# kirilllzaitsev/vision_mtl

Hardware: AMD Instinct MI355X
Metric: images/sec fwd+bwd, basic model 128x256 (higher is better)
Workload: dtype f32

## Files before the change

### include/vmtl.h

```cpp
#ifndef VMTL_H
#define VMTL_H

#ifdef __cplusplus
extern "C" {
#endif

#define VMTL_ACT_NONE 0
#define VMTL_ACT_RELU 1
#define VMTL_ACT_HSWISH 2
#define VMTL_ACT_HSIGMOID 3
#define VMTL_ACT_SIGMOID 4

#define VMTL_PREC_FP32 0
#define VMTL_PREC_BF16 1

const char* vmtl_version(void);
const char* vmtl_last_error_string(void);
int vmtl_reload_env(void);
int vmtl_timestamp(long long* out, void* stream);


int vmtl_conv2d_fwd(const float* x, const float* wp, const float* bias, float* y, float* stats,
                    int B, int H, int W, int Cs, int Ho, int Wo, int ldy, int Nw, int Cout,
                    int KH, int KW, int stride, int pad, int act, int shuffle, void* stream);
// ... 34 lines not shown
                           const float* ez_x, const float* ez_mean, const float* ez_invstd, const float* ez_gamma,
                           const float* ez_beta, int ez_act, int M, int Ks, int ldy, int Nw, int Cout, void* stream);

int vmtl_conv2d_bnbwd(const float* x, const float* wp, float* y, float* stats, const float* ez_x, const float* ez_mean,
                      const float* ez_invstd, const float* ez_gamma, const float* ez_beta, int ez_act, int B, int H,
                      int W, int Cs, int Ho, int Wo, int ldy, int Nw, int Cout, int KH, int KW, int stride, int pad,
                      void* stream);
int vmtl_conv2d_bnbwd_p(const float* x, const float* wp, float* y, float* stats, const float* ez_x, const float* ez_mean,
                        const float* ez_invstd, const float* ez_gamma, const float* ez_beta, int ez_act, int B, int H,
                        int W, int Cs, int Ho, int Wo, int ldy, int Nw, int Cout, int KH, int KW, int stride, int pad,
                        int precision, void* stream);

int vmtl_conv2d_up2_fwd(const float* xl, const float* skip, const float* wp_eff, float* y, float* stats,
                        int B, int H2, int W2, int C0s, int C1s, int ldy, int Cout, void* stream);
int vmtl_conv2d_up2_fwd_p(const float* xl, const float* skip, const float* wp_eff, float* y, float* stats,
                          int B, int H2, int W2, int C0s, int C1s, int ldy, int Cout, int precision, void* stream);
int vmtl_conv2d_up2_stats_block(int B, int H2, int W2, int ldy);
int vmtl_conv2d_up2_ksplit(int B, int H2, int W2, int ldy, int Ktot);
int vmtl_conv2d_up2_fwd_ws(const float* xl, const float* skip, const float* wp_eff, float* y, float* ws, int B, int H2,
                           int W2, int C0s, int C1s, int ldy, int Cout, void* stream);
int vmtl_conv2d_up2_fwd_ws_p(const float* xl, const float* skip, const float* wp_eff, float* y, float* ws, int B, int H2,
                             int W2, int C0s, int C1s, int ldy, int Cout, int precision, void* stream);
int vmtl_conv2d_up2_halo(const float* xl, const float* skip, const float* wp_eff, float* y, float* stats,
                         int B, int H2, int W2, int C0s, int C1s, int ldy, int Cout, void* stream);
int vmtl_conv2d_up2_halo_supported(int B, int H2, int W2, int C0s, int C1s, int ldy, int Cout);
int vmtl_conv2d_up2_halo_stat_rows(int B, int H2, int W2, int C0s, int C1s, int ldy, int Cout);
int vmtl_conv2d_up2_halo_stat_block(int C0s, int C1s, int ldy, int Cout);
int vmtl_pack_up2_fwd(const float* w, float* dst, int Cout, int C0, int C0s, int C1, int C1s, void* stream);
int vmtl_pack_up2_dgrad(const float* w, float* dst, int Cout, int Cos, int C0, int Cin, void* stream);
int vmtl_unpack_up2(const float* slabs, float* grad, int Cout, int Cos, int C0, int Cin, int nslabs, void* stream);

int vmtl_conv2d_wgrad_splits(int M, int Nw, int Ktot);
int vmtl_conv2d_wgrad(const float* x, const float* dy, float* slabs, int splits, int B, int H, int W, int Cs,
                      int Ho, int Wo, int ldy, int Nw, int KH, int KW, int stride, int pad, void* stream);
int vmtl_conv2d_wgrad_p(const float* x, const float* dy, float* slabs, int splits, int B, int H, int W, int Cs,
                        int Ho, int Wo, int ldy, int Nw, int KH, int KW, int stride, int pad, int precision,
                        void* stream);

int vmtl_conv3x3_wgrad_small_supported(int Cs, int ldy, int W);
int vmtl_conv3x3_wgrad_small_slabs(int B, int H, int W);
int vmtl_conv3x3_wgrad_small(const float* x, const float* dy, float* slabs, int nslabs, int B, int H, int W, int Cs,
                             int ldy, int Nw, void* stream);


int vmtl_conv3x3_small_supported(int Cs, int Nw);
int vmtl_conv3x3_small_tiles(int B, int H, int W);
int vmtl_conv3x3_small_stat_rows(int B, int H, int W);
int vmtl_conv3x3_small_stat_block(int B, int H, int W);
int vmtl_conv3x3_small(const float* x, const float* x2, const float* pa, const float* pb, const float* pc,
                       int act_in, float* a_out, const float* wp, const float* bias, float* y, float* yb, int Ca,
                       float* stats, int ep_mode, const float* ez_x, const float* ez_mean, const float* ez_invstd,
                       const float* ez_gamma, const float* ez_beta, int ez_act, int B, int H, int W, int Cs, int ldy,
                       int Nw, int Cout, void* stream);

int vmtl_dwconv_fwd(const float* x, const float* wp, float* y, int B, int H, int W, int Cs, int Ho, int Wo,
                    int K, int stride, int pad, void* stream);
int vmtl_dwconv_bn_stats_rows(int M, int Cs);
int vmtl_dwconv_bn_stats_block(int M, int Cs);
int vmtl_dwconv_bn_fwd(const float* x, const float* coef_a, const float* coef_c, int act, const float* wp, float* y,
                       float* a_out, float* partial, int B, int H, int W, int Cs, int Ho, int Wo, int K, int stride,
                       int pad, void* stream);
int vmtl_dwconv_bwd_data(const float* dy, const float* wp, float* dx, int B, int H, int W, int Cs, int Ho,
                         int Wo, int K, int stride, int pad, void* stream);
int vmtl_dwconv_bwd_data_add(const float* dy, const float* wp, const float* addend, float* dx, int B, int H, int W,
                             int Cs, int Ho, int Wo, int K, int stride, int pad, void* stream);
int vmtl_dwconv_bwd_weight_rows(int M, int Cs);
int vmtl_dwconv_bwd_weight(const float* x, const float* dy, float* partial, float* dw, int B, int H, int W,
                           int C, int Cs, int Ho, int Wo, int K, int stride, int pad, void* stream);

int vmtl_pack_weights(const float* src, float* dst, int R1, int R0, int T, int C, int Cs, long long sr1,
                      long long sr0, long long st, long long sc, int flip, void* stream);
int vmtl_pack_weights_scaled(const float* src, float* dst, int R1, int R0, int T, int C, int Cs, long long sr1,
                             long long sr0, long long st, long long sc, int flip, const float* scale, int sstride,
                             int smode, void* stream);
int vmtl_unpack_weights_stitch(const float* packed, float* grad, const float* w, const float* scale, int sstride,
                               float* ds, float* work, int R0, int T, int C, int Cs, int nslabs, long long slab_stride,
                               int reduce_all, void* stream);
int vmtl_pack_desc_bytes(void);
int vmtl_pack_weights_batch(const void* descs, int n, long long total, void* stream);
int vmtl_pack_weights_slice(const float* src, float* dst, int R0, int T, int C, int group, long long sr0,
                            long long st, long long sc, int flip, void* stream);
int vmtl_unpack_weights(const float* packed, float* grad, int R1, int R0, int T, int C, int Cs,
                        long long sr1, long long sr0, long long st, long long sc, int flip, int nslabs,
                        long long slab_stride, void* stream);

int vmtl_reduce_rows(int M);
int vmtl_bn_stats(const float* x, int M, int C, int Cs, float* partial, int nblk_from_conv,
                  int rows_per_blk_from_conv, float eps, float momentum, float* running_mean, float* running_var, long long* num_batches_tracked,
                  float* save_mean, float* save_invstd, void* stream);
int vmtl_bn_eval_stats(const float* running_mean, const float* running_var, int C, int Cs, float eps,
                       float* save_mean, float* save_invstd, void* stream);
int vmtl_bn_stats_coef(const float* x, int M, int C, int Cs, float* partial, int nblk_from_conv,
                       int rows_per_blk_from_conv, float eps, float momentum, float* running_mean, float* running_var,
                       long long* num_batches_tracked, float* save_mean, float* save_invstd, const float* gamma,
                       const float* beta, float* coef_a, float* coef_c, void* stream);
int vmtl_bn_eval_stats_coef(const float* running_mean, const float* running_var, int C, int Cs, float eps,
                            float* save_mean, float* save_invstd, const float* gamma, const float* beta,
                            float* coef_a, float* coef_c, void* stream);
int vmtl_bn_apply(const float* x, const float* mean, const float* invstd, const float* gamma,
                  const float* beta, const float* mul, const float* res, float* y, long long M, int C,
                  int Cs, int act, void* stream);
int vmtl_bn_fuse_max_rows(void);
int vmtl_bn_apply_fused(const float* x, const float* partial, int nblk, int rows_per_blk, float eps, float momentum,
                        float* running_mean, float* running_var, long long* num_batches_tracked, float* save_mean,
                        float* save_invstd, const float* gamma, const float* beta, const float* mul, const float* res,
                        float* y, long long M, int C, int Cs, int act, void* stream);
// ... 93 lines not shown
```

### vision_mtl_amd/ops.py

```python
from __future__ import annotations

import contextlib
import os
import weakref

import torch

from ._lib import lib
from .precision import conv_prec_code

ACT_NONE, ACT_RELU, ACT_HSWISH, ACT_HSIGMOID, ACT_SIGMOID = 0, 1, 2, 3, 4
ACT_CODES = {None: 0, "none": 0, "relu": 1, "hardswish": 2, "hardsigmoid": 3, "sigmoid": 4}


def ceil4(c: int) -> int:
    return (c + 3) // 4 * 4


def _stream() -> int:
    return torch.cuda.current_stream().cuda_stream


def _req(t: torch.Tensor, name: str = "tensor") -> torch.Tensor:
    if not t.is_cuda:
# ... 371 lines not shown


FUSE_DW = os.environ.get("VMTL_FUSE_DW", "1") != "0"
_PW = os.environ.get("VMTL_PW", "1") != "0"
_PW_MAX_ROWS = int(os.environ.get("VMTL_PW_MAX_ROWS", str(1 << 21)))


_UP2_HALO = os.environ.get("VMTL_UP2_HALO", "1") != "0"


def _up2_halo_route(B, H2, W2, C0s, C1s, ldy, Cout, prec) -> bool:
    return (_UP2_HALO and prec == 0 and bool(lib().raw("vmtl_conv2d_up2_halo_supported")(B, H2, W2, C0s, C1s, ldy, Cout))
            and lib().raw("vmtl_conv2d_up2_ksplit")(B, H2, W2, ldy, 4 * C0s + 9 * C1s) == 1)


def up2_stats_geometry(B, H2, W2, C0s, C1s, ldy, Cout, prec=None):
    prec = conv_prec_code() if prec is None else prec
    if _up2_halo_route(B, H2, W2, C0s, C1s, ldy, Cout, prec):
        return (lib().raw("vmtl_conv2d_up2_halo_stat_rows")(B, H2, W2, C0s, C1s, ldy, Cout),
                lib().raw("vmtl_conv2d_up2_halo_stat_block")(C0s, C1s, ldy, Cout))
    if lib().raw("vmtl_conv2d_up2_ksplit")(B, H2, W2, ldy, 4 * C0s + 9 * C1s) > 1:
        return 0, 0
    bm = lib().raw("vmtl_conv2d_up2_stats_block")(B, H2, W2, ldy)
    Mq = B * H2 * W2
    return (4 * (Mq // bm), bm) if Mq % bm == 0 else (0, bm)


def _is_pw(B, Ho, Wo, KH, KW, stride, pad, shuffle=0):
    return _PW and KH == 1 and KW == 1 and stride == 1 and pad == 0 and not shuffle and B * Ho * Wo <= _PW_MAX_ROWS


_SMALL_MIN_ROWS = int(os.environ.get("VMTL_SMALL_MIN_ROWS", str(1 << 16)))


def conv_ksplit(B, Ho, Wo, Cs, ldy, KH, KW, stride, pad, shuffle=0) -> int:
    if shuffle or _is_pw(B, Ho, Wo, KH, KW, stride, pad, shuffle):
        return 1
    return lib().raw("vmtl_conv2d_ksplit")(B, Ho, Wo, ldy, KH * KW * Cs)


_SMALL_STATS = os.environ.get("VMTL_SMALL_STATS", "1") != "0"


def _small_route(B, H, W, Cs, ldy, KH, KW, stride, pad, shuffle=0, with_stats=False) -> bool:
    if shuffle or KH != 3 or KW != 3 or stride != 1 or pad != 1 or ldy > 36 or B * H * W < _SMALL_MIN_ROWS:
        return False
    if B * H * W * 36 > 0x7FFFFFFF:
        return False
    if not conv3x3_small_supported(Cs, ldy):
        return False
    return not with_stats or (_SMALL_STATS and H % 4 == 0 and W % 32 == 0)


def conv_stats_geometry(B, Ho, Wo, Cs, ldy, KH, KW, stride, pad):
    if _small_route(B, Ho, Wo, Cs, ldy, KH, KW, stride, pad, with_stats=True):
        return lib().raw("vmtl_conv3x3_small_stat_rows")(B, Ho, Wo), lib().raw("vmtl_conv3x3_small_stat_block")(B, Ho, Wo)
    if _is_pw(B, Ho, Wo, KH, KW, stride, pad):
        M = B * Ho * Wo
        return lib().raw("vmtl_conv1x1_stats_rows")(M, ldy, Cs, 0), lib().raw("vmtl_conv1x1_stats_block")(M, ldy, Cs, 0)
    return lib().raw("vmtl_conv2d_stats_rows")(B, Ho, Wo, ldy), lib().raw("vmtl_conv2d_stats_block")(B, Ho, Wo, ldy)


def _conv_launch(x, wp, bias, y, stats, B, H, W, Cs, Ho, Wo, ldy, Nw, Cout, KH, KW, stride, pad, shuffle=0, cin=None,
                 algo_flop=None, prec=0):
    flop = 2.0 * B * Ho * Wo * Nw * KH * KW * (Cs if cin is None else cin)
    if _is_pw(B, Ho, Wo, KH, KW, stride, pad, shuffle):
        _k("vmtl_conv1x1_fwd", _flop=flop if algo_flop is None else algo_flop, _xflop=flop, x=x, wp=wp, bias=bias, y=y,
           stats=stats, M=B * Ho * Wo, Ks=Cs, ldy=ldy, Nw=Nw, Cout=Cout)
        return
    if _small_route(B, H, W, Cs, ldy, KH, KW, stride, pad, shuffle, with_stats=stats is not None):
        _small(x, wp, y, B, H, W, Cs, ldy, Nw, Cout, flop if algo_flop is None else algo_flop, bias=bias, stats=stats,
               ep_mode=1 if stats is not None else 0)
        return
    if stats is None and not shuffle:
        ks = lib().raw("vmtl_conv2d_ksplit")(B, Ho, Wo, ldy, KH * KW * Cs)
        if ks > 1:
            ws = _empty((ks, B * Ho * Wo, ldy), x)
            _kp("vmtl_conv2d_fwd_ws", prec, _flop=flop if algo_flop is None else algo_flop, _xflop=flop, x=x, wp=wp, bias=bias, y=y,
               ws=ws, B=B, H=H, W=W, Cs=Cs, Ho=Ho, Wo=Wo, ldy=ldy, Nw=Nw, Cout=Cout, KH=KH, KW=KW, stride=stride, pad=pad)
            return
    _kp("vmtl_conv2d_fwd", prec, _flop=flop if algo_flop is None else algo_flop, _xflop=flop, x=x, wp=wp, bias=bias, y=y, stats=stats, B=B, H=H, W=W, Cs=Cs, Ho=Ho, Wo=Wo, ldy=ldy,
       Nw=Nw, Cout=Cout, KH=KH, KW=KW, stride=stride, pad=pad, act=0, shuffle=shuffle)


def _stitch_view(stitch_w, task, C):
    T = stitch_w.shape[0]
    if stitch_w.dim() == 3:
        if stitch_w.shape[2] != C:
            raise ValueError(f"stitched conv: the stitch layer has {stitch_w.shape[2]} channels, the conv reads {C}")
        return (task * T + task) * C, 1
    return task * T + task, 0


class _Conv2d(torch.autograd.Function):

    @staticmethod
    def forward(ctx, x, weight, bias, stride, pad, want_stats, zero_bias_grad=False, stitch_w=None, stitch_task=0):
        x = _req(x, "x")
        weight = _req(weight, "weight")
        B, H, W, Cs = x.shape
        Cout, Cin, KH, KW = weight.shape
        if ceil4(Cin) != Cs:
            raise ValueError(f"conv2d: input has {Cs} storage channels, weight expects Cin={Cin}")
        KK = KH * KW
        Ho = (H + 2 * pad - KH) // stride + 1
        Wo = (W + 2 * pad - KW) // stride + 1
        ldy = ceil4(Cout)
        if stitch_w is None:
            wp = packs.get(weight, "fwd", (1, Cout, KK, Cin, Cs, 0, Cin * KK, 1, KK, 0))
        else:
            stitch_w = _req(stitch_w, "stitch weights")
            soff, sstride = _stitch_view(stitch_w, stitch_task, Cin)
            wp = packs.get(weight, f"fwd_st{stitch_task}", (1, Cout, KK, Cin, Cs, 0, Cin * KK, 1, KK, 0),
                           scale=(stitch_w, soff, sstride, 1))
        y = _empty((B, Ho, Wo, ldy), x)
        stats = None
        if want_stats and conv_ksplit(B, Ho, Wo, Cs, ldy, KH, KW, stride, pad) > 1:
            want_stats = False
        if want_stats:
            rows, _ = conv_stats_geometry(B, Ho, Wo, Cs, ldy, KH, KW, stride, pad)
            stats = _empty((rows, 2, ldy), x)
        prec = ctx.prec = conv_prec_code()
        _conv_launch(x, wp, bias, y, stats, B, H, W, Cs, Ho, Wo, ldy, Cout, Cout, KH, KW, stride, pad, cin=Cin, prec=prec)
        ctx.save_for_backward(x, weight, stitch_w)
        ctx.cfg = (stride, pad, bias is not None)
# ... 306 lines not shown

    @staticmethod
    def backward(ctx, dy, _dstats):
        xl, skip, weight = ctx.saved_tensors
        C0, C1, _ = ctx.cfg
        if dy is None:
            return None, None, None, None
        dy = _req(dy, "dy")
        B, H2, W2, C0s = xl.shape
        Cout, Cin = weight.shape[0], weight.shape[1]
        H, W, ldy = 2 * H2, 2 * W2, dy.shape[3]
        dxl = dskip = dw = None
        stamp(f"main up2 M={B * H * W} N={Cout} Cin={Cin}")
        fork = side.mark()
        if ctx.needs_input_grad[0]:
            wd = packs.get_custom(weight, "up2_dgrad", (C0, 16 * ldy), lambda w, dst: _k(
                "vmtl_pack_up2_dgrad", w=w, dst=dst, Cout=Cout, Cos=ldy, C0=C0, Cin=Cin))
            dxl = _empty((B, H2, W2, C0s), xl)
            _conv_launch(dy, wd, None, dxl, None, B, H, W, ldy, H2, W2, C0s, C0, C0, 4, 4, 2, 1, cin=Cout,
                         algo_flop=2.0 * B * H * W * C0 * 9 * Cout, prec=ctx.prec)
        if skip is not None and ctx.needs_input_grad[1]:
            C1s = skip.shape[3]
            wds = packs.get(weight, "up2_dskip", (1, C1, 9, Cout, ldy, 0, 9, 1, Cin * 9, 1), offset=C0 * 9)
            dskip = _empty((B, H, W, C1s), xl)
            _conv_launch(dy, wds, None, dskip, None, B, H, W, ldy, H, W, C1s, C1, C1, 3, 3, 1, 1, cin=Cout, prec=ctx.prec)
        if ctx.needs_input_grad[2]:
            dw = _empty(weight.shape, xl) if ctx.slot is None else ctx.slot
            with side.branch(ctx.slot is not None, B * H * W, fork, dy, xl, skip):
                slabs, ns = _wgrad(dy, xl, B, H, W, ldy, H2, W2, C0s, C0, 4, 4, 2, 1, 2.0 * B * H * W * Cout * 9 * C0,
                                   xflop=2.0 * B * H2 * W2 * C0 * 16 * Cout, prec=ctx.prec)
                _k("vmtl_unpack_up2", slabs=slabs, grad=dw, Cout=Cout, Cos=ldy, C0=C0, Cin=Cin, nslabs=ns)
                if skip is not None:
                    C1s = skip.shape[3]
                    slabs, ns = _wgrad(skip, dy, B, H, W, C1s, H, W, ldy, Cout, 3, 3, 1, 1,
                                       2.0 * B * H * W * Cout * 9 * C1, prec=ctx.prec)
                    unpack(slabs, None, 1, Cout, 9, C1, C1s, 0, Cin * 9, 1, 9, out=dw.view(-1)[C0 * 9:], nslabs=ns)
                stamp(f"side up2 M={B * H * W} N={Cout} Cin={Cin}")
            if ctx.slot is not None:
                dw = None
        return dxl, dskip, dw, None, None


class _BNActConv(torch.autograd.Function):

    @staticmethod
    def forward(ctx, x, stats, rpb, gamma, beta, rm, rv, nbt, weight, skip, cfg):
        C, training, momentum, eps, act, up2, want_stats = cfg
        x, weight = _req(x, "x"), _req(weight, "weight")
        B, H, W, Cs = x.shape
        M = B * H * W
        Cout, Cin = weight.shape[0], weight.shape[1]
        if ceil4(C) != Cs or tuple(weight.shape[2:]) != (3, 3):
            raise ValueError("bn_act_conv: 3x3 weight over x's channels expected")
        mean, invstd = _empty((Cs,), x), _empty((Cs,), x)
        a = _empty(x.shape, x)
        if training:
            if stats is not None:
                partial, nblk = stats, stats.shape[0]
            else:
                partial, nblk, rpb = _empty((_reduce_rows(M), 2, Cs), x), 0, 0
            if 0 < nblk <= _BN_FUSE_ROWS:
                _k("vmtl_bn_apply_fused", x=x, partial=partial, nblk=nblk, rows_per_blk=rpb, eps=eps, momentum=momentum,
                   running_mean=rm, running_var=rv, num_batches_tracked=nbt, save_mean=mean, save_invstd=invstd,
                   gamma=gamma, beta=beta, mul=None, res=None, y=a, M=M, C=C, Cs=Cs, act=act)
            else:
                _k("vmtl_bn_stats", x=x, M=M, C=C, Cs=Cs, partial=partial, nblk_from_conv=nblk, rows_per_blk_from_conv=rpb,
                   eps=eps, momentum=momentum, running_mean=rm, running_var=rv, num_batches_tracked=nbt, save_mean=mean,
                   save_invstd=invstd)
                _k("vmtl_bn_apply", x=x, mean=mean, invstd=invstd, gamma=gamma, beta=beta, mul=None, res=None, y=a, M=M,
                   C=C, Cs=Cs, act=act)
        else:
            _k("vmtl_bn_eval_stats", running_mean=rm, running_var=rv, C=C, Cs=Cs, eps=eps, save_mean=mean, save_invstd=invstd)
            _k("vmtl_bn_apply", x=x, mean=mean, invstd=invstd, gamma=gamma, beta=beta, mul=None, res=None, y=a, M=M, C=C,
               Cs=Cs, act=act)
        prec = ctx.prec = conv_prec_code()
        ldy = ceil4(Cout)
        ostats, orpb = None, 0
        if up2:
            if skip is not None:
                skip = _req(skip, "skip")
                C1s = skip.shape[3]
                if tuple(skip.shape[:3]) != (B, 2 * H, 2 * W):
                    raise ValueError("bn_act_conv(up2): skip must be at twice the resolution of x")
            else:
                C1s = 0
            C1 = Cin - C
            if ceil4(C1) != C1s or (C1 > 0) != (skip is not None):
                raise ValueError("bn_act_conv(up2): weight channels do not match x + skip")
            Ktot = 4 * Cs + 9 * C1s
            wp = packs.get_custom(weight, "up2_fwd", (4, Cout, Ktot), lambda w, dst: _k(
                "vmtl_pack_up2_fwd", w=w, dst=dst, Cout=Cout, C0=C, C0s=Cs, C1=C1, C1s=C1s))
            y = _empty((B, 2 * H, 2 * W, ldy), x)
            Mo = 4 * M
            ks = lib().raw("vmtl_conv2d_up2_ksplit")(B, H, W, ldy, Ktot)
            if _up2_halo_route(B, H, W, Cs, C1s, ldy, Cout, prec):
                if want_stats:
                    rows, bm = up2_stats_geometry(B, H, W, Cs, C1s, ldy, Cout, prec)
                    if rows:
                        ostats, orpb = _empty((rows, 2, ldy), x), bm
                _k("vmtl_conv2d_up2_halo", _flop=2.0 * Mo * Cout * 9 * Cin, _xflop=2.0 * Mo * Cout * (4 * C + 9 * C1), xl=a,
                   skip=skip, wp_eff=wp, y=y, stats=ostats, B=B, H2=H, W2=W, C0s=Cs, C1s=C1s, ldy=ldy, Cout=Cout)
            elif ks > 1:
                _kp("vmtl_conv2d_up2_fwd_ws", prec, _flop=2.0 * Mo * Cout * 9 * Cin, _xflop=2.0 * Mo * Cout * (4 * C + 9 * C1),
                   xl=a, skip=skip, wp_eff=wp, y=y, ws=_empty((ks, B, 2 * H, 2 * W, ldy), x), B=B, H2=H, W2=W, C0s=Cs,
                   C1s=C1s, ldy=ldy, Cout=Cout)
            else:
                if want_stats:
                    bm = lib().raw("vmtl_conv2d_up2_stats_block")(B, H, W, ldy)
                    if M % bm == 0:
                        ostats, orpb = _empty((4 * (M // bm), 2, ldy), x), bm
                _kp("vmtl_conv2d_up2_fwd", prec, _flop=2.0 * Mo * Cout * 9 * Cin, _xflop=2.0 * Mo * Cout * (4 * C + 9 * C1), xl=a,
                   skip=skip, wp_eff=wp, y=y, stats=ostats, B=B, H2=H, W2=W, C0s=Cs, C1s=C1s, ldy=ldy, Cout=Cout)
        else:
            if Cin != C or skip is not None:
                raise ValueError("bn_act_conv: weight expects x's channels (skip only with up2)")
            wp = packs.get(weight, "fwd", (1, Cout, 9, Cin, Cs, 0, Cin * 9, 1, 9, 0))
            y = _empty((B, H, W, ldy), x)
            if want_stats and conv_ksplit(B, H, W, Cs, ldy, 3, 3, 1, 1) == 1:
                rows, orpb = conv_stats_geometry(B, H, W, Cs, ldy, 3, 3, 1, 1)
                ostats = _empty((rows, 2, ldy), x)
            _conv_launch(a, wp, None, y, ostats, B, H, W, Cs, H, W, ldy, Cout, Cout, 3, 3, 1, 1, cin=Cin, prec=prec)
        ctx.save_for_backward(x, a, skip, weight, mean, invstd, gamma, beta)
        ctx.cfg = (C, training, act, up2)
        ctx.slots = (_slot(gamma), _slot(beta), _slot(weight))
        ctx.orpb = orpb
        ctx.set_materialize_grads(False)
        if ostats is not None:
            ctx.mark_non_differentiable(ostats)
        return y, ostats

    @staticmethod
    def backward(ctx, dy, _dstats):
        x, a, skip, weight, mean, invstd, gamma, beta = ctx.saved_tensors
        C, training, act, up2 = ctx.cfg
        sg, sb, sw = ctx.slots
        if dy is None:
            return (None,) * 11
        dy = _req(dy, "dy")
        B, H, W, Cs = x.shape
        M = B * H * W
        Cout, Cin = weight.shape[0], weight.shape[1]
        ldy = dy.shape[3]
        stamp(f"main bnconv M={dy.shape[0] * dy.shape[1] * dy.shape[2]} N={Cout} Cin={Cin}")
        fork = side.mark()
        if up2:
            Hd, Wd = 2 * H, 2 * W
            wd = packs.get_custom(weight, "up2_dgrad", (C, 16 * ldy), lambda w, dst: _k(
                "vmtl_pack_up2_dgrad", w=w, dst=dst, Cout=Cout, Cos=ldy, C0=C, Cin=Cin))
            geo = dict(B=B, H=Hd, W=Wd, Cs=ldy, Ho=H, Wo=W, ldy=Cs, Nw=C, Cout=C, KH=4, KW=4, stride=2, pad=1)
            flop, xflop = 2.0 * B * Hd * Wd * C * 9 * Cout, 2.0 * M * C * 16 * Cout
        else:
            Hd, Wd = H, W
            wd = packs.get(weight, "dgrad", (1, Cin, 9, Cout, ldy, 0, 9, 1, Cin * 9, 1))
            geo = dict(B=B, H=H, W=W, Cs=ldy, Ho=H, Wo=W, ldy=Cs, Nw=Cin, Cout=Cin, KH=3, KW=3, stride=1, pad=1)
            flop = xflop = 2.0 * M * Cin * 9 * Cout
        dgamma = _empty((C,), x) if sg is None else sg
        dbeta = _empty((C,), x) if sb is None else sb
        dx = _empty(x.shape, x) if ctx.needs_input_grad[0] else None
        fuse = lib().raw("vmtl_conv2d_ksplit")(B, H, W, Cs, geo["KH"] * geo["KW"] * ldy) <= 1 \
            and os.environ.get("VMTL_BNBWD_FUSE", "1") != "0"
        if fuse:
            dz = _empty(x.shape, x)
            if not up2 and _small_route(B, H, W, ldy, Cs, 3, 3, 1, 1, with_stats=True):
                rows = lib().raw("vmtl_conv3x3_small_stat_rows")(B, H, W)
                part = _empty((rows, 2, Cs), x)
                _small(dy, wd, dz, B, H, W, ldy, Cs, Cin, Cin, flop, stats=part, ep_mode=2,
                       ez=(x, mean, invstd, gamma, beta, act))
            else:
                rows = lib().raw("vmtl_conv2d_stats_rows")(B, H, W, Cs)
                part = _empty((rows, 2, Cs), x)
                _kp("vmtl_conv2d_bnbwd", ctx.prec, _flop=flop, _xflop=xflop, x=dy, wp=wd, y=dz, stats=part, ez_x=x, ez_mean=mean,
                   ez_invstd=invstd, ez_gamma=gamma, ez_beta=beta, ez_act=act, **geo)
            _k("vmtl_bn_bwd_finalize", partial=part, nblk=rows, M=M, C=C, Cs=Cs, sum_dz=dbeta, sum_dzx=dgamma, mean=None,
               invstd=None, gamma=None, training=1 if training else 0, coef_a=None, coef_b=None, coef_c=None)
            if dx is not None:
                _k("vmtl_bn_bwd_apply", x=x, dz=dz, mean=mean, invstd=invstd, gamma=gamma, sum_dz=dbeta, sum_dzx=dgamma,
                   dx=dx, M=M, C=C, Cs=Cs, training=1 if training else 0)
        else:
            da = _empty(x.shape, x)
            _conv_launch(dy, wd, None, da, None, geo["B"], geo["H"], geo["W"], geo["Cs"], geo["Ho"], geo["Wo"], geo["ldy"],
                         geo["Nw"], geo["Cout"], geo["KH"], geo["KW"], geo["stride"], geo["pad"], cin=Cout, algo_flop=flop,
                         prec=ctx.prec)
            part = _empty((_reduce_rows(M), 2, Cs), x)
            _k("vmtl_bn_bwd", x=x, dy=da, mean=mean, invstd=invstd, gamma=gamma, beta=beta, mul=None, dmul=None,
               partial=part, sum_dz=dbeta, sum_dzx=dgamma, dx=dx if dx is not None else _empty(x.shape, x), M=M, C=C, Cs=Cs,
               act=act, training=1 if training else 0)
        dskip = None
        if up2 and skip is not None and ctx.needs_input_grad[9]:
            C1, C1s = Cin - C, skip.shape[3]
            wds = packs.get(weight, "up2_dskip", (1, C1, 9, Cout, ldy, 0, 9, 1, Cin * 9, 1), offset=C * 9)
            dskip = _empty(skip.shape, x)
            _conv_launch(dy, wds, None, dskip, None, B, Hd, Wd, ldy, Hd, Wd, C1s, C1, C1, 3, 3, 1, 1, cin=Cout, prec=ctx.prec)
        dw = _empty(weight.shape, x) if sw is None else sw
        with side.branch(sw is not None, B * Hd * Wd, fork, dy, a, skip):
            if up2:
                slabs, ns = _wgrad(dy, a, B, Hd, Wd, ldy, H, W, Cs, C, 4, 4, 2, 1, 2.0 * B * Hd * Wd * Cout * 9 * C,
                                   xflop=2.0 * M * C * 16 * Cout, prec=ctx.prec)
                _k("vmtl_unpack_up2", slabs=slabs, grad=dw, Cout=Cout, Cos=ldy, C0=C, Cin=Cin, nslabs=ns)
                if skip is not None:
                    C1, C1s = Cin - C, skip.shape[3]
                    slabs, ns = _wgrad(skip, dy, B, Hd, Wd, C1s, Hd, Wd, ldy, Cout, 3, 3, 1, 1,
                                       2.0 * B * Hd * Wd * Cout * 9 * C1, prec=ctx.prec)
                    unpack(slabs, None, 1, Cout, 9, C1, C1s, 0, Cin * 9, 1, 9, out=dw.view(-1)[C * 9:], nslabs=ns)
            else:
                slabs, ns = _wgrad(a, dy, B, H, W, Cs, H, W, ldy, Cout, 3, 3, 1, 1, 2.0 * M * Cout * 9 * Cin, prec=ctx.prec)
                unpack(slabs, weight.shape, 1, Cout, 9, Cin, Cs, 0, Cin * 9, 1, 9, out=dw, nslabs=ns)
            stamp(f"side bnconv N={Cout} Cin={Cin}")
        nif = lambda g, slot: None if slot is not None else g
        return dx, None, None, nif(dgamma, sg), nif(dbeta, sb), None, None, None, nif(dw, sw), dskip, None


def bn_act_conv(x, stats, rpb, bn, C, act, weight, skip=None, up2=False, want_stats=True):
    if bn.momentum is None:
        raise NotImplementedError("BatchNorm2d(momentum=None) (cumulative moving average) is not implemented")
    cfg = (C, bn.training, float(bn.momentum), bn.eps, act, bool(up2), bool(want_stats))
    y, ostats = _BNActConv.apply(x, stats, rpb, bn.weight, bn.bias, bn.running_mean, bn.running_var,
                                 bn.num_batches_tracked, weight, skip, cfg)
    orpb = 0
    if ostats is not None:
        B, H, W, _ = x.shape
# ... 1173 lines not shown
```

Measured before the change: 2592.

## Add halo-tiled MFMA 3x3 conv kernel with fused BN prologue and stats epilogue

Adds a new 3x3 stride-1 conv kernel for 64/68 input channels. It stages a haloed 4x32 pixel tile of the input in LDS, runs fp32 MFMA with a software-pipelined weight prefetch, and writes BN statistics or the BN-backward dz epilogue from the output tile. The BN->act->conv forward path now applies the BN affine and ReLU inside the conv prologue and writes the activation as a side output, which removes the separate bn_apply pass. The kernel is routed for mid-size fp32 convs in forward, the generic conv launcher and BN backward. In exchange it adds a large new code path with several template variants and extra LDS use.

```diff
diff --git a/include/vmtl.h b/include/vmtl.h
--- a/include/vmtl.h
+++ b/include/vmtl.h
@@ -110,6 +110,14 @@
                        float* stats, int ep_mode, const float* ez_x, const float* ez_mean, const float* ez_invstd,
                        const float* ez_gamma, const float* ez_beta, int ez_act, int B, int H, int W, int Cs, int ldy,
                        int Nw, int Cout, void* stream);
+
+int vmtl_conv3x3_halo_supported(int B, int H, int W, int Cs, int ldy, int Nw);
+int vmtl_conv3x3_halo_stat_rows(int B, int H, int W);
+int vmtl_conv3x3_halo_stat_block(int B, int H, int W);
+int vmtl_conv3x3_halo(const float* x, const float* pa, const float* pc, int act_in, float* a_out, const float* wp,
+                      const float* bias, float* y, float* stats, int ep_mode, const float* ez_x, const float* ez_mean,
+                      const float* ez_invstd, const float* ez_gamma, const float* ez_beta, int ez_act, int B, int H,
+                      int W, int Cs, int ldy, int Nw, int Cout, void* stream);
 
 int vmtl_dwconv_fwd(const float* x, const float* wp, float* y, int B, int H, int W, int Cs, int Ho, int Wo,
                     int K, int stride, int pad, void* stream);
diff --git a/vision_mtl_amd/csrc/conv3x3_halo.hip b/vision_mtl_amd/csrc/conv3x3_halo.hip
--- /dev/null
+++ b/vision_mtl_amd/csrc/conv3x3_halo.hip
@@ -0,0 +1,392 @@
+#include "common.h"
+
+#define CH_TM 4
+#define CH_TW 32
+#define CH_HX (CH_TW + 2)
+#define CH_NHALO ((CH_TM + 2) * CH_HX)
+#define CH_NP (CH_NHALO | 1)
+#define CH_NPX (CH_TM * CH_TW)
+
+struct HaloP {
+  const float* x;
+  const float* pa;
+  const float* pc;
+  float* a_out;
+  const float* wp;
+  const float* bias;
+  float* y;
+  float* stats;
+  const float* ez_x;
+  const float* ez_mean;
+  const float* ez_invstd;
+  const float* ez_gamma;
+  const float* ez_beta;
+  int act_in, ep_mode, ez_act;
+  int B, H, W, ldy, Nw, Cout;
+  int tiles_x, tiles_y;
+  unsigned x_bytes, wp_bytes;
+};
+
+template <int CS, int TN, bool TAIL>
+struct HaloCfg {
+  static constexpr int SP = CS / 4, FG = SP / 4, RS = SP % 4;
+  static constexpr int KQ = 9 * SP;
+  static constexpr int NGF = 9 * FG, NR = 9 * RS, NGR = (NR + 3) / 4;
+  static constexpr int NG = NGF + NGR;
+  static constexpr int NROWS = 16 * TN;
+  static constexpr int OS = NROWS + 4;
+  static constexpr int SQ = TAIL ? OS / 4 : TN * 4;
+  static constexpr int NRT = 2 * CH_TM;
+  static constexpr int WM = 4 / TN;
+  static constexpr int RT = NRT / WM;
+  static constexpr int NST = CH_NHALO * SP;
+  static constexpr int IT = (NST + 255) / 256;
+  static constexpr int ZQ = SP * CH_NP;
+  static constexpr int HALO4 = ZQ + 1;
+  static constexpr int OT4 = CH_NPX * OS / 4;
+  static constexpr int RED4 = 2 * 256;
+  static constexpr int MAIN4 = HALO4 > OT4 + RED4 ? HALO4 : OT4 + RED4;
+  static constexpr int PQ = (OS + 3) / 4;
+  static constexpr int PAR4 = 2 * SP + 5 * PQ;
+  static constexpr int LDS_BYTES = (MAIN4 + PAR4) * 16;
+  static_assert(TN == 1 || TN == 2 || TN == 4, "column tiles");
+  static_assert(!TAIL || TN == 4, "tail columns only next to 4 MFMA column tiles (one per wave)");
+  static_assert(CS % 4 == 0 && FG >= 1, "channel quads");
+};
+
+__device__ __forceinline__ f32x4 ch_bload(__amdgpu_buffer_rsrc_t r, unsigned off) {
+  return __builtin_bit_cast(f32x4, __builtin_amdgcn_raw_buffer_load_b128(r, off, 0, 0));
+}
+
+template <int CS, int TN, bool TAIL>
+__global__ __launch_bounds__(256) __attribute__((amdgpu_waves_per_eu(2))) void conv3x3_halo_kernel(HaloP p) {
+  using C = HaloCfg<CS, TN, TAIL>;
+  constexpr int SP = C::SP, FG = C::FG, RS = C::RS, KQ = C::KQ, NGF = C::NGF, NR = C::NR, NGR = C::NGR, NG = C::NG;
+  constexpr int NROWS = C::NROWS, OS = C::OS, RT = C::RT, IT = C::IT, ZQ = C::ZQ, PQ = C::PQ;
+  constexpr int NB = TAIL ? 2 : 1;
+  constexpr unsigned OOB = 0xFFFFFFFFu;
+
+  extern __shared__ __attribute__((aligned(16))) f32x4 smem4[];
+  f32x4* halo = smem4;
+  float* otile = reinterpret_cast<float*>(smem4);
+  f32x4* red = smem4 + C::OT4;
+  f32x4* par = smem4 + C::MAIN4;
+  f32x4* epar = par + 2 * SP;
+
+  const int tid = threadIdx.x;
+  const int lane = tid & 63, wv = __builtin_amdgcn_readfirstlane(tid >> 6);
+  const int l15 = lane & 15, lq = lane >> 4;
+  const int jw = wv % TN, rw = wv / TN;
+
+  int t = blockIdx.x;
+  const int tx = t % p.tiles_x;
+  t /= p.tiles_x;
+  const int ty = t % p.tiles_y, b = t / p.tiles_y;
+  const int h0 = ty * CH_TM, w0 = tx * CH_TW;
+
+  const __amdgpu_buffer_rsrc_t rs_x = __builtin_amdgcn_make_buffer_rsrc((void*)p.x, 0, p.x_bytes, 0x00020000);
+  const __amdgpu_buffer_rsrc_t rs_w = __builtin_amdgcn_make_buffer_rsrc((void*)p.wp, 0, p.wp_bytes, 0x00020000);
+
+  const bool has_pro = p.pa != nullptr;
+  if (tid < 2 * SP) {
+    const float* src = tid < SP ? p.pa : p.pc;
+    const int s = tid < SP ? tid : tid - SP;
+    par[tid] = has_pro ? *reinterpret_cast<const f32x4*>(src + 4 * s) : (f32x4){0.f, 0.f, 0.f, 0.f};
+  }
+  if (tid < 5 * PQ) {
+    const int which = tid / PQ, q = tid - which * PQ;
+    const float* src = which == 0 ? p.bias : (which == 1 ? p.ez_mean : (which == 2 ? p.ez_invstd : (which == 3 ? p.ez_gamma : p.ez_beta)));
+    f32x4 v = {0.f, 0.f, 0.f, 0.f};
+    if (src != nullptr && (which == 0 || p.ep_mode == 2)) {
+#pragma unroll
+      for (int e = 0; e < 4; ++e)
+        if (4 * q + e < p.Cout) v[e] = src[4 * q + e];
+    }
+    epar[tid] = v;
+  }
+
+  unsigned wrow[NB];
+  {
+    const int n = 16 * jw + l15;
+    wrow[0] = n < p.Nw ? (unsigned)(n * KQ) * 16u : 0x80000000u;
+    if (TAIL) {
+      const int nt = NROWS + wv;
+      wrow[NB - 1] = nt < p.Nw ? (unsigned)(nt * KQ) * 16u : 0x80000000u;
+    }
+  }
+  int arem[NGR > 0 ? NGR : 1];
+  unsigned krem[NGR > 0 ? NGR : 1];
+#pragma unroll
+  for (int h = 0; h < NGR; ++h) {
+    const int r = 4 * h + lq;
+    if (r < NR) {
+      const int tap = r / (RS > 0 ? RS : 1), s = FG * 4 + r % (RS > 0 ? RS : 1);
+      arem[h] = s * CH_NP + (tap / 3) * CH_HX + tap % 3 + l15;
+      krem[h] = (unsigned)(tap * SP + s) * 16u;
+    } else {
+      arem[h] = -1;
+      krem[h] = 0x40000000u;
+    }
+  }
+  const int a0 = lq * CH_NP + l15;
+  auto rtoff = [](int i) { return (i >> 1) * CH_HX + 16 * (i & 1); };
+
+  {
+    f32x4 r0[IT];
+#pragma unroll
+    for (int it = 0; it < IT; ++it) {
+      const int f = tid + 256 * it;
+      const int pp = f / SP, s = f - pp * SP;
+      const int hy = pp / CH_HX, hx = pp - hy * CH_HX;
+      const int gh = h0 - 1 + hy, gw = w0 - 1 + hx;
+      const bool ok = f < C::NST && (unsigned)gh < (unsigned)p.H && (unsigned)gw < (unsigned)p.W;
+      r0[it] = ch_bload(rs_x, ok ? (unsigned)((b * p.H + gh) * p.W + gw) * (unsigned)(CS * 4) + 16u * s : OOB);
+    }
+    if (has_pro) __syncthreads();
+#pragma unroll
+    for (int it = 0; it < IT; ++it) {
+      const int f = tid + 256 * it;
+      if (f >= C::NST) continue;
+      const int pp = f / SP, s = f - pp * SP;
+      f32x4 v = r0[it];
+      if (has_pro) {
+        const int hy = pp / CH_HX, hx = pp - hy * CH_HX;
+        const int gh = h0 - 1 + hy, gw = w0 - 1 + hx;
+        const bool ok = (unsigned)gh < (unsigned)p.H && (unsigned)gw < (unsigned)p.W;
+        v = v * par[s] + par[SP + s];
+        if (p.act_in == VMTL_ACT_RELU) {
+#pragma unroll
+          for (int e = 0; e < 4; ++e) v[e] = fmaxf(v[e], 0.f);
+        }
+        if (!ok) v = (f32x4){0.f, 0.f, 0.f, 0.f};
+        if (p.a_out != nullptr && ok && hy >= 1 && hy <= CH_TM && hx >= 1 && hx <= CH_TW)
+          *reinterpret_cast<f32x4*>(p.a_out + (size_t)((b * p.H + gh) * p.W + gw) * CS + 4 * s) = v;
+      }
+      halo[s * CH_NP + pp] = v;
+    }
+    if (tid == 0) halo[ZQ] = (f32x4){0.f, 0.f, 0.f, 0.f};
+  }
+
+  constexpr int SQ = C::SQ, G = 256 / SQ;
+  constexpr int EIT = (CH_NPX + G - 1) / G;
+  const int eq = tid % SQ, gi = tid / SQ;
+  const bool elane = gi < G;
+  f32x4 rz[EIT];
+  if (p.ep_mode == 2) {
+#pragma unroll
+    for (int it = 0; it < EIT; ++it) {
+      const int px = gi + it * G;
+      const int gy = h0 + px / CH_TW, gx = w0 + px % CH_TW;
+      rz[it] = (f32x4){0.f, 0.f, 0.f, 0.f};
+      if (elane && px < CH_NPX && gy < p.H && gx < p.W)
+        rz[it] = *reinterpret_cast<const f32x4*>(p.ez_x + (size_t)((b * p.H + gy) * p.W + gx) * p.ldy + 4 * eq);
+    }
+  }
+  __syncthreads();
+
+  f32x4 acc[RT];
+  f32x2 tacc[TAIL ? C::NRT : 1];
+#pragma unroll
+  for (int i = 0; i < RT; ++i) acc[i] = (f32x4){0.f, 0.f, 0.f, 0.f};
+#pragma unroll
+  for (int i = 0; i < (TAIL ? C::NRT : 1); ++i) tacc[i] = (f32x2){0.f, 0.f};
+  const int rbase = rw * RT;
+  auto group = [&](int g, unsigned& koff, int& ai) {
+    if (g < NGF) {
+      const int tap = g / FG, cb = (g % FG) * 4;
+      koff = (unsigned)(tap * SP + cb + lq) * 16u;
+      ai = a0 + cb * CH_NP + (tap / 3) * CH_HX + tap % 3;
+    } else {
+      koff = krem[g - NGF];
+      ai = arem[g - NGF];
+    }
+  };
+  auto load_b = [&](int g, f32x4 (&bq)[NB]) {
+    unsigned koff;
+    int ai;
+    group(g, koff, ai);
+#pragma unroll
+    for (int j = 0; j < NB; ++j) bq[j] = ch_bload(rs_w, wrow[j] + koff);
+  };
+  auto load_a = [&](int g, f32x4 (&aq)[RT]) {
+    unsigned koff;
+    int ai;
+    group(g, koff, ai);
+#pragma unroll
+    for (int i = 0; i < RT; ++i) aq[i] = halo[ai < 0 ? ZQ : ai + rtoff(rbase + i)];
+  };
+  auto mma = [&](const f32x4 (&aq)[RT], const f32x4 (&bq)[NB]) {
+#pragma unroll
+    for (int e = 0; e < 4; ++e)
+#pragma unroll
+      for (int i = 0; i < RT; ++i) acc[i] = __builtin_amdgcn_mfma_f32_16x16x4f32(aq[i][e], bq[0][e], acc[i], 0, 0, 0);
+    if (TAIL) {
+      const f32x4 w = bq[NB - 1];
+      const f32x2 lo = __builtin_shufflevector(w, w, 0, 1), hi = __builtin_shufflevector(w, w, 2, 3);
+#pragma unroll
+      for (int i = 0; i < (TAIL ? C::NRT : 1); ++i) {
+        tacc[i] += __builtin_shufflevector(aq[i], aq[i], 0, 1) * lo;
+        tacc[i] += __builtin_shufflevector(aq[i], aq[i], 2, 3) * hi;
+        asm volatile("" : "+v"(tacc[i]));
+      }
+    }
+  };
+  f32x4 bq[3][NB], aq[2][RT];
+  load_b(0, bq[0]);
+  if (NG > 1) load_b(1, bq[1]);
+  load_a(0, aq[0]);
+#pragma unroll
+  for (int g = 0; g < NG; ++g) {
+    if (g + 2 < NG) load_b(g + 2, bq[(g + 2) % 3]);
+    if (g + 1 < NG) load_a(g + 1, aq[(g + 1) & 1]);
+    mma(aq[g & 1], bq[g % 3]);
+    if (g + 2 < NG) __builtin_amdgcn_sched_group_barrier(0x020, NB, 0);
+    if (g + 1 < NG) __builtin_amdgcn_sched_group_barrier(0x100, RT, 0);
+    __builtin_amdgcn_sched_group_barrier(0x008, 4 * RT, 0);
+    if (TAIL) __builtin_amdgcn_sched_group_barrier(0x002, 4 * C::NRT + 8, 0);
+    __builtin_amdgcn_sched_barrier(0);
+  }
+
+  float tv[TAIL ? C::NRT : 1];
+  if (TAIL) {
+#pragma unroll
+    for (int i = 0; i < (TAIL ? C::NRT : 1); ++i) tv[i] = quarter_sum(tacc[i][0] + tacc[i][1]);
+  }
+  __syncthreads();
+#pragma unroll
+  for (int i = 0; i < RT; ++i) {
+    const int px0 = 16 * (rbase + i) + 4 * lq;
+#pragma unroll
+    for (int r = 0; r < 4; ++r) otile[(px0 + r) * OS + 16 * jw + l15] = acc[i][r];
+  }
+  if (TAIL && lq == 0) {
+#pragma unroll
+    for (int i = 0; i < (TAIL ? C::NRT : 1); ++i) otile[(16 * i + l15) * OS + NROWS + wv] = tv[i];
+  }
+  __syncthreads();
+
+  const f32x4* ot4 = reinterpret_cast<const f32x4*>(otile);
+  constexpr int SQS = OS / 4;
+  f32x4 val[EIT];
+  f32x4 s1 = {0.f, 0.f, 0.f, 0.f}, s2 = s1;
+#pragma unroll
+  for (int it = 0; it < EIT; ++it) {
+    const int px = gi + it * G;
+    val[it] = (f32x4){0.f, 0.f, 0.f, 0.f};
+    if (elane && px < CH_NPX) {
+      f32x4 v = ot4[px * SQS + eq];
+      const int gy = h0 + px / CH_TW, gx = w0 + px % CH_TW;
+      const bool ok = gy < p.H && gx < p.W;
+      if (p.ep_mode == 2) {
+        const f32x4 xh = (rz[it] - epar[PQ + eq]) * epar[2 * PQ + eq];
+        const f32x4 z = epar[3 * PQ + eq] * xh + epar[4 * PQ + eq];
+#pragma unroll
+        for (int e = 0; e < 4; ++e) v[e] *= act_grad(z[e], p.ez_act);
+        if (!ok) v = (f32x4){0.f, 0.f, 0.f, 0.f};
+        s1 += v;
+        s2 += v * xh;
+      } else {
+        v += epar[eq];
+        if (ok) s1 += v;
+      }
+      val[it] = v;
+      if (ok) *reinterpret_cast<f32x4*>(p.y + (size_t)((b * p.H + gy) * p.W + gx) * p.ldy + 4 * eq) = v;
+    }
+  }
+
+  if (p.ep_mode != 0) {
+    red[tid] = s1;
+    red[256 + tid] = s2;
+    __syncthreads();
+    f32x4* srow = reinterpret_cast<f32x4*>(p.stats + (size_t)blockIdx.x * 2 * p.ldy);
+    if (p.ep_mode == 1) {
+      f32x4 m = {0.f, 0.f, 0.f, 0.f};
+      for (int k = 0; k < G; ++k) m += red[k * SQ + eq];
+      m *= 1.f / (float)CH_NPX;
+      f32x4 c = {0.f, 0.f, 0.f, 0.f};
+#pragma unroll
+      for (int it = 0; it < EIT; ++it)
+        if (elane && gi + it * G < CH_NPX) c += (val[it] - m) * (val[it] - m);
+      red[256 + tid] = c;
+      __syncthreads();
+      if (tid < SQ) {
+        f32x4 m2 = {0.f, 0.f, 0.f, 0.f};
+        for (int k = 0; k < G; ++k) m2 += red[256 + k * SQ + tid];
+        srow[tid] = m;
+        srow[SQ + tid] = m2;
+      }
+    } else if (tid < SQ) {
+      f32x4 a = {0.f, 0.f, 0.f, 0.f}, c = a;
+      for (int k = 0; k < G; ++k) {
+        a += red[k * SQ + tid];
+        c += red[256 + k * SQ + tid];
+      }
+      srow[tid] = a;
+      srow[SQ + tid] = c;
+    }
+  }
+}
+
+template <int CS, int TN, bool TAIL>
+static int launch_halo(HaloP& p, hipStream_t st) {
+  using C = HaloCfg<CS, TN, TAIL>;
+  static_assert(C::LDS_BYTES * 2 <= 160 * 1024, "two workgroups per CU");
+  if (hipFuncSetAttribute(reinterpret_cast<const void*>(&conv3x3_halo_kernel<CS, TN, TAIL>),
+                          hipFuncAttributeMaxDynamicSharedMemorySize, C::LDS_BYTES) != hipSuccess)
+    return VMTL_ERR_LAUNCH;
+  p.tiles_x = cdiv(p.W, CH_TW);
+  p.tiles_y = cdiv(p.H, CH_TM);
+  hipLaunchKernelGGL((conv3x3_halo_kernel<CS, TN, TAIL>), dim3(p.B * p.tiles_x * p.tiles_y), dim3(256), C::LDS_BYTES, st, p);
+  return vmtl_check_launch();
+}
+
+static int halo_tn(int ldy) {
+  return ldy == 16 ? 1 : (ldy == 32 ? 2 : (ldy == 64 || ldy == 68 ? 4 : 0));
+}
+
+extern "C" int vmtl_conv3x3_halo_supported(int B, int H, int W, int Cs, int ldy, int Nw) {
+  if (B <= 0 || H <= 0 || W <= 0 || (Cs != 64 && Cs != 68) || halo_tn(ldy) == 0 || Nw < 1 || ((Nw + 3) & ~3) != ldy)
+    return 0;
+  return (long long)B * H * W * Cs * 4 <= 0x7fffffffLL;
+}
+
+extern "C" int vmtl_conv3x3_halo_stat_rows(int B, int H, int W) {
+  if (B <= 0 || H <= 0 || W <= 0 || H % CH_TM || W % CH_TW) return 0;
+  return B * (H / CH_TM) * (W / CH_TW);
+}
+
+extern "C" int vmtl_conv3x3_halo_stat_block(int B, int H, int W) {
+  return vmtl_conv3x3_halo_stat_rows(B, H, W) > 0 ? CH_NPX : 0;
+}
+
+extern "C" int vmtl_conv3x3_halo(const float* x, const float* pa, const float* pc, int act_in, float* a_out,
+                                 const float* wp, const float* bias, float* y, float* stats, int ep_mode,
+                                 const float* ez_x, const float* ez_mean, const float* ez_invstd, const float* ez_gamma,
+                                 const float* ez_beta, int ez_act, int B, int H, int W, int Cs, int ldy, int Nw,
+                                 int Cout, void* stream) {
+  VMTL_ENTER();
+  if (!x || !wp || !y || B <= 0 || H <= 0 || W <= 0 || Cout <= 0 || Cout > Nw) return VMTL_ERR_ARG;
+  if ((pa == nullptr) != (pc == nullptr) || (a_out != nullptr && pa == nullptr)) return VMTL_ERR_ARG;
+  if (act_in != VMTL_ACT_NONE && act_in != VMTL_ACT_RELU) return VMTL_ERR_ARG;
+  if (ep_mode < 0 || ep_mode > 2 || (ep_mode != 0 && !stats) || (ep_mode == 0 && stats)) return VMTL_ERR_ARG;
+  if (ep_mode != 0 && vmtl_conv3x3_halo_stat_rows(B, H, W) == 0) return VMTL_ERR_ARG;
+  if (ep_mode == 2 && (!ez_x || !ez_mean || !ez_invstd || !ez_gamma || !ez_beta || bias)) return VMTL_ERR_ARG;
+  if (!vmtl_conv3x3_halo_supported(B, H, W, Cs, ldy, Nw)) return VMTL_ERR_UNSUPPORTED;
+  HaloP p;
+  p.x = x; p.pa = pa; p.pc = pc; p.a_out = a_out; p.wp = wp; p.bias = bias; p.y = y; p.stats = stats;
+  p.ez_x = ez_x; p.ez_mean = ez_mean; p.ez_invstd = ez_invstd; p.ez_gamma = ez_gamma; p.ez_beta = ez_beta;
+  p.act_in = act_in; p.ep_mode = ep_mode; p.ez_act = ez_act;
+  p.B = B; p.H = H; p.W = W; p.ldy = ldy; p.Nw = Nw; p.Cout = Cout;
+  p.x_bytes = (unsigned)((long long)B * H * W * Cs * 4);
+  p.wp_bytes = (unsigned)(Nw * 9 * Cs * 4);
+  hipStream_t st = (hipStream_t)stream;
+  const int tn = halo_tn(ldy);
+  if (Cs == 68) {
+    if (tn == 1) return launch_halo<68, 1, false>(p, st);
+    if (tn == 2) return launch_halo<68, 2, false>(p, st);
+    return ldy == 64 ? launch_halo<68, 4, false>(p, st) : launch_halo<68, 4, true>(p, st);
+  }
+  if (tn == 1) return launch_halo<64, 1, false>(p, st);
+  if (tn == 2) return launch_halo<64, 2, false>(p, st);
+  return ldy == 64 ? launch_halo<64, 4, false>(p, st) : launch_halo<64, 4, true>(p, st);
+}
diff --git a/vision_mtl_amd/ops.py b/vision_mtl_amd/ops.py
--- a/vision_mtl_amd/ops.py
+++ b/vision_mtl_amd/ops.py
@@ -447,9 +447,34 @@
     return not with_stats or (_SMALL_STATS and H % 4 == 0 and W % 32 == 0)
 
 
+_MID_HALO = os.environ.get("VMTL_MID_HALO", "1") != "0"
+_MID_HALO_MIN_ROWS = int(os.environ.get("VMTL_MID_HALO_MIN_ROWS", str(1 << 16)))
+
+
+def _mid_halo_route(B, H, W, Cs, ldy, KH, KW, stride, pad, shuffle=0, with_stats=False, prec=None) -> bool:
+    prec = conv_prec_code() if prec is None else prec
+    if not _MID_HALO or prec != 0 or shuffle or KH != 3 or KW != 3 or stride != 1 or pad != 1 or B * H * W < _MID_HALO_MIN_ROWS:
+        return False
+    if not lib().raw("vmtl_conv3x3_halo_supported")(B, H, W, Cs, ldy, ldy):
+        return False
+    if lib().raw("vmtl_conv2d_ksplit")(B, H, W, ldy, 9 * Cs) > 1:
+        return False
+    return not with_stats or lib().raw("vmtl_conv3x3_halo_stat_rows")(B, H, W) > 0
+
+
+def _mid_halo(x, wp, y, B, H, W, Cs, ldy, Nw, Cout, flop, pa=None, pc=None, act_in=ACT_NONE, a_out=None, bias=None,
+              stats=None, ep_mode=0, ez=None):
+    ez = ez or (None, None, None, None, None, ACT_NONE)
+    _k("vmtl_conv3x3_halo", _flop=flop, x=x, pa=pa, pc=pc, act_in=act_in, a_out=a_out, wp=wp, bias=bias, y=y, stats=stats,
+       ep_mode=ep_mode, ez_x=ez[0], ez_mean=ez[1], ez_invstd=ez[2], ez_gamma=ez[3], ez_beta=ez[4], ez_act=ez[5], B=B, H=H,
+       W=W, Cs=Cs, ldy=ldy, Nw=Nw, Cout=Cout)
+
+
 def conv_stats_geometry(B, Ho, Wo, Cs, ldy, KH, KW, stride, pad):
     if _small_route(B, Ho, Wo, Cs, ldy, KH, KW, stride, pad, with_stats=True):
         return lib().raw("vmtl_conv3x3_small_stat_rows")(B, Ho, Wo), lib().raw("vmtl_conv3x3_small_stat_block")(B, Ho, Wo)
+    if _mid_halo_route(B, Ho, Wo, Cs, ldy, KH, KW, stride, pad, with_stats=True):
+        return lib().raw("vmtl_conv3x3_halo_stat_rows")(B, Ho, Wo), lib().raw("vmtl_conv3x3_halo_stat_block")(B, Ho, Wo)
     if _is_pw(B, Ho, Wo, KH, KW, stride, pad):
         M = B * Ho * Wo
         return lib().raw("vmtl_conv1x1_stats_rows")(M, ldy, Cs, 0), lib().raw("vmtl_conv1x1_stats_block")(M, ldy, Cs, 0)
@@ -466,6 +491,10 @@
     if _small_route(B, H, W, Cs, ldy, KH, KW, stride, pad, shuffle, with_stats=stats is not None):
         _small(x, wp, y, B, H, W, Cs, ldy, Nw, Cout, flop if algo_flop is None else algo_flop, bias=bias, stats=stats,
                ep_mode=1 if stats is not None else 0)
+        return
+    if _mid_halo_route(B, H, W, Cs, ldy, KH, KW, stride, pad, shuffle, with_stats=stats is not None, prec=prec):
+        _mid_halo(x, wp, y, B, H, W, Cs, ldy, Nw, Cout, flop if algo_flop is None else algo_flop, bias=bias, stats=stats,
+                  ep_mode=1 if stats is not None else 0)
         return
     if stats is None and not shuffle:
         ks = lib().raw("vmtl_conv2d_ksplit")(B, Ho, Wo, ldy, KH * KW * Cs)
@@ -878,9 +907,15 @@
         Cout, Cin = weight.shape[0], weight.shape[1]
         if ceil4(C) != Cs or tuple(weight.shape[2:]) != (3, 3):
             raise ValueError("bn_act_conv: 3x3 weight over x's channels expected")
-        mean, invstd = _empty((Cs,), x), _empty((Cs,), x)
+        prec = ctx.prec = conv_prec_code()
+        ldy = ceil4(Cout)
+        pro = (not up2 and skip is None and Cin == C and act in (ACT_NONE, ACT_RELU)
+               and _mid_halo_route(B, H, W, Cs, ldy, 3, 3, 1, 1, with_stats=want_stats, prec=prec))
         a = _empty(x.shape, x)
-        if training:
+        if pro:
+            mean, invstd, ca, cc = _bn_fwd_coef(x, stats, rpb, gamma, beta, rm, rv, nbt, C, training, momentum, eps)
+        elif training:
+            mean, invstd = _empty((Cs,), x), _empty((Cs,), x)
             if stats is not None:
                 partial, nblk = stats, stats.shape[0]
             else:
@@ -896,11 +931,10 @@
                 _k("vmtl_bn_apply", x=x, mean=mean, invstd=invstd, gamma=gamma, beta=beta, mul=None, res=None, y=a, M=M,
                    C=C, Cs=Cs, act=act)
         else:
+            mean, invstd = _empty((Cs,), x), _empty((Cs,), x)
             _k("vmtl_bn_eval_stats", running_mean=rm, running_var=rv, C=C, Cs=Cs, eps=eps, save_mean=mean, save_invstd=invstd)
             _k("vmtl_bn_apply", x=x, mean=mean, invstd=invstd, gamma=gamma, beta=beta, mul=None, res=None, y=a, M=M, C=C,
                Cs=Cs, act=act)
-        prec = ctx.prec = conv_prec_code()
-        ldy = ceil4(Cout)
         ostats, orpb = None, 0
         if up2:
             if skip is not None:
@@ -945,7 +979,11 @@
             if want_stats and conv_ksplit(B, H, W, Cs, ldy, 3, 3, 1, 1) == 1:
                 rows, orpb = conv_stats_geometry(B, H, W, Cs, ldy, 3, 3, 1, 1)
                 ostats = _empty((rows, 2, ldy), x)
-            _conv_launch(a, wp, None, y, ostats, B, H, W, Cs, H, W, ldy, Cout, Cout, 3, 3, 1, 1, cin=Cin, prec=prec)
+            if pro:
+                _mid_halo(x, wp, y, B, H, W, Cs, ldy, Cout, Cout, 2.0 * M * Cout * 9 * Cin, pa=ca, pc=cc, act_in=act, a_out=a,
+                          stats=ostats, ep_mode=1 if ostats is not None else 0)
+            else:
+                _conv_launch(a, wp, None, y, ostats, B, H, W, Cs, H, W, ldy, Cout, Cout, 3, 3, 1, 1, cin=Cin, prec=prec)
         ctx.save_for_backward(x, a, skip, weight, mean, invstd, gamma, beta)
         ctx.cfg = (C, training, act, up2)
         ctx.slots = (_slot(gamma), _slot(beta), _slot(weight))
@@ -992,6 +1030,11 @@
                 part = _empty((rows, 2, Cs), x)
                 _small(dy, wd, dz, B, H, W, ldy, Cs, Cin, Cin, flop, stats=part, ep_mode=2,
                        ez=(x, mean, invstd, gamma, beta, act))
+            elif not up2 and _mid_halo_route(B, H, W, ldy, Cs, 3, 3, 1, 1, with_stats=True, prec=ctx.prec):
+                rows = lib().raw("vmtl_conv3x3_halo_stat_rows")(B, H, W)
+                part = _empty((rows, 2, Cs), x)
+                _mid_halo(dy, wd, dz, B, H, W, ldy, Cs, Cin, Cin, flop, stats=part, ep_mode=2,
+                          ez=(x, mean, invstd, gamma, beta, act))
             else:
                 rows = lib().raw("vmtl_conv2d_stats_rows")(B, H, W, Cs)
                 part = _empty((rows, 2, Cs), x)
```

Result: faster. 2641, median of 6 (+1.9%).
